# jcbowden/EagleEverything

Measured on NVIDIA B200. Metric: markers/s, higher is better.
Workload: dtype f64

## Files before the change

eagleeverything_b200/csrc/capi.cu:

```cuda
#include <cublas_v2.h>
#include <dlfcn.h>
#include <fcntl.h>
#include <sys/mman.h>
#include <sys/stat.h>
#include <unistd.h>

#include <cmath>
#include <cstdarg>
#include <cstdlib>
#include <cstring>
#include <atomic>
#include <condition_variable>
#include <functional>
#include <mutex>
#include <thread>
#include <unordered_map>
#include <string>
#include <vector>

#include "common.cuh"
#include "hostio.cuh"

struct eg_store {
    int8_t* d = nullptr;
// ... 82 lines not shown
    if (g_ctx.ready) return check_cuda(cudaSetDevice(g_ctx.device), "cudaSetDevice");
    const char* env = getenv("EAGLE_GPU_DEVICE");
    return eg_init(env ? atoi(env) : 0);
}

int ensure_init_pub() { return ensure_init(); }
cudaStream_t ctx_stream() { return g_ctx.stream; }
cublasHandle_t ctx_cublas() { return g_ctx.cublas; }

void syrk_release_cache();
void scan_i8_release();
void algebra_release();
void eigbasis_release();
void prep_i8_release();
int launch_prepare_i8(const double* d_S, const double* d_V, int64_t n, int64_t col0, int64_t col1, double* d_tmp,
                      double* d_Wp, int64_t Kpad, cudaStream_t st, bool* done);
static int g_scan_mode = -1;
int scan_mode() {
    if (g_scan_mode < 0) {
        const char* e = getenv("EAGLE_SCAN_MODE");
        g_scan_mode = (e && (e[0] == 'f' || e[0] == 'd' || e[0] == '0')) ? 0 : 1;
    }
    return g_scan_mode;
}
int launch_scan(const int8_t* d_Mt, int64_t L, int64_t n, int64_t pitch, const double* d_Wp,
                const int64_t* d_zero_rows, int n_zero, double* d_a, double* d_vara, cudaStream_t st);

static void pool_flush_locked() {
    for (auto& b : g_ctx.free_blocks) cudaFreeAsync(b.p, g_ctx.stream);
    g_ctx.free_blocks.clear();
    g_ctx.free_bytes = 0;
// ... 422 lines not shown
    __shared__ int8_t tile[32][33];
    const int tx = threadIdx.x & 31, ty = threadIdx.x >> 5;
    const int64_t r0 = (int64_t)blockIdx.y * 32, c0 = (int64_t)blockIdx.x * 32;
    for (int i = ty; i < 32; i += 8) {
        const int64_t r = r0 + i, c = c0 + tx;
        tile[i][tx] = (r < rows && c < cols) ? in[r * pitch + c] : (int8_t)0;
    }
    __syncthreads();
    for (int i = ty; i < 32; i += 8) {
        const int64_t c = c0 + i, r = r0 + tx;
        if (r < rows && c < cols) out[r + c * rows] = -(double)tile[tx][i];
    }
}

__global__ void __launch_bounds__(256) symmetrize_upper_kernel(double* __restrict__ Wp, int64_t n, int64_t ld,
                                                               int w_is_upper) {
    __shared__ double tile[32][33];
    const int bx = blockIdx.x, by = blockIdx.y;
    if (bx < by) return;
    const int tx = threadIdx.x & 31, ty = threadIdx.x >> 5;
    const int64_t r0 = (int64_t)by * 32, c0 = (int64_t)bx * 32;
    for (int i = ty; i < 32; i += 8) {
        const int64_t r = c0 + tx, c = r0 + i;
        tile[i][tx] = (r < n && c < n) ? Wp[r + c * ld] : 0.0;
    }
    __syncthreads();
    for (int i = ty; i < 32; i += 8) {
        const int64_t r = r0 + tx, c = c0 + i;
        if (r < n && c < n) {
            if (r < c) Wp[r + c * ld] = Wp[r + c * ld] + (w_is_upper ? Wp[r + c * ld] : tile[tx][i]);
            else if (r > c) Wp[r + c * ld] = 0.0;
        }
    }
    if (bx != by) {
        __syncthreads();
        for (int i = ty; i < 32; i += 8) {
            const int64_t r = c0 + tx, c = r0 + i;
            if (r < n && c < n) Wp[r + c * ld] = 0.0;
        }
    }
}

__global__ void __launch_bounds__(256) symmetry_kernel(const double* __restrict__ A, int64_t n,
                                                       unsigned long long* __restrict__ out) {
    __shared__ double tile[64][65];
// ... 25 lines not shown
            const double a = v[k], b = tile[tx][i];
            mabs = fmax(mabs, fmax(fabs(a), fabs(b)));
            const double d = fabs(a - b);
            masym = fmax(masym, d == d ? d : 1.0e300);
        }
    }
#pragma unroll
    for (int o = 16; o > 0; o >>= 1) {
        mabs = fmax(mabs, __shfl_xor_sync(0xffffffffu, mabs, o));
        masym = fmax(masym, __shfl_xor_sync(0xffffffffu, masym, o));
    }
    if ((threadIdx.x & 31) == 0) {
        atomicMax(out, (unsigned long long)__double_as_longlong(mabs));
        atomicMax(out + 1, (unsigned long long)__double_as_longlong(masym));
    }
}

static void say(eg_message_fn message, void* ctx, const char* fmt, ...) {
    if (!message) return;
    char buf[512];
    va_list ap;
    va_start(ap, fmt);
    vsnprintf(buf, sizeof(buf), fmt, ap);
    va_end(ap);
    message(ctx, buf);
}

}

using namespace eg;
// ... 371 lines not shown
    MTRACE("scan: upload of 1/%d of S and V", N);
    EG_TRY(agree(upload()));
    if (N > 1) {
        EG_NCCL(g_nccl.GroupStart());
        for (int q = 0; q < N; q++) {
            int64_t q0, q1;
            shard_range(n, N, q, 1, &q0, &q1);
            if (q1 == q0) continue;
            EG_NCCL(g_nccl.Broadcast(dS.as<double>() + q0 * n, dS.as<double>() + q0 * n, (size_t)(q1 - q0) * n, NCCL_FLOAT64, q, g_multi.comm[r], st));
            EG_NCCL(g_nccl.Broadcast(dV.as<double>() + q0 * n, dV.as<double>() + q0 * n, (size_t)(q1 - q0) * n, NCCL_FLOAT64, q, g_multi.comm[r], st));
        }
        EG_NCCL(g_nccl.GroupEnd());
    }
    g_ctx.timing[4] = t_up.stop();
    Timer t_prep(st);
    int sym = 0;
    bool split = false;
    std::vector<int64_t> cuts(N + 1, n);
    auto products = [&]() -> int {
        EG_TRY(eg_dev_inputs_symmetric(dS.as<double>(), dV.as<double>(), n, &sym, st));
        split = sym && eg_prep_uses_i8(n);
        for (int q = 0; q < N; q++) {
            if (split) {
                int64_t c = (int64_t)llround((double)n * (sqrt(1.0 + 3.0 * q / N) - 1.0) / 32.0) * 32;
                cuts[q] = c < n ? c : n;
            } else {
                cuts[q] = q == 0 ? 0 : n;
            }
        }
        int64_t widest = 1;
        for (int q = 0; q < N; q++) widest = std::max(widest, cuts[q + 1] - cuts[q]);
        EG_TRY(dT.alloc((size_t)n * (split ? widest : n) * 8, "scan scratch"));
        EG_CUDA(cudaMemsetAsync(dW.p, 0, (size_t)eg_scan_wp_elems(n) * 8, st));
        return eg_dev_scan_prepare_cols(dS.as<double>(), dV.as<double>(), n, split ? cuts[r] : 0, split ? cuts[r + 1] : n, sym,
                                        dT.as<double>(), dW.as<double>(), st);
    };
    MTRACE("scan: pre-products of my columns of W");
    EG_TRY(agree(products()));
    if (N > 1) {
        EG_NCCL(g_nccl.GroupStart());
        for (int q = 0; q < N && split; q++)
            if (cuts[q + 1] > cuts[q])
                EG_NCCL(g_nccl.Broadcast(dW.as<double>() + cuts[q] * Kpad, dW.as<double>() + cuts[q] * Kpad,
                                         (size_t)(cuts[q + 1] - cuts[q]) * Kpad, NCCL_FLOAT64, q, g_multi.comm[r], st));
        EG_NCCL(g_nccl.GroupEnd());
    }
    EG_TRY(eg_dev_scan_fold(dS.as<double>(), da.as<double>(), n, sym, dW.as<double>(), st));
    g_ctx.timing[5] = t_prep.stop();
    MTRACE("scan: %lld markers", (long long)L);
    if (L > 0) {
        const std::vector<int64_t> z = slot_indices(Mt, r, zero_rows);
        {
            Timer t(st);
            EG_TRY(eg_dev_scan(part->d, L, n, part->pitch, dW.as<double>(), z.empty() ? nullptr : z.data(), (int64_t)z.size(),
                               oa.as<double>(), ov.as<double>(), st));
            g_ctx.timing[6] = t.stop();
        }
        Timer t(st);
        EG_CUDA(cudaMemcpyAsync(out_a + Mt->off[r], oa.p, (size_t)L * 8, cudaMemcpyDeviceToHost, st));
        EG_CUDA(cudaMemcpyAsync(out_vara + Mt->off[r], ov.p, (size_t)L * 8, cudaMemcpyDeviceToHost, st));
        EG_CUDA(cudaStreamSynchronize(st));
        g_ctx.timing[7] = t.stop();
// ... 373 lines not shown
    if (env_pm && env_pm[0] == 'f') return 0;
    return n >= 512;
}

extern "C" int eg_dev_scan_prepare_cols(const double* d_S, const double* d_V, int64_t n, int64_t col0, int64_t col1,
                                        int upper_only, double* d_tmp, double* d_Wp, void* stream) {
    if (!d_S || !d_V || !d_tmp || !d_Wp || n <= 0 || col0 < 0 || col1 > n || col0 > col1)
        return set_error(EG_ERR_ARG, "eg_dev_scan_prepare_cols: bad argument");
    if (col0 == col1) return EG_OK;
    EG_TRY(ensure_init());
    cudaStream_t st = (cudaStream_t)stream;
    const int64_t Kpad = round_up(n, 32), nc = col1 - col0;
    const bool want_i8 = eg_prep_uses_i8(n) != 0;
    if (upper_only && want_i8) {
        bool done = false;
        EG_TRY(launch_prepare_i8(d_S, d_V, n, col0, col1, d_tmp, d_Wp, Kpad, st, &done));
        if (done) return EG_OK;
    }
    const double one = 1.0, zero = 0.0;
    if (cublasSetStream(g_ctx.cublas, st) != CUBLAS_STATUS_SUCCESS) return set_error(EG_ERR_CUDA, "cublasSetStream");
    if (cublasDgemm(g_ctx.cublas, CUBLAS_OP_N, CUBLAS_OP_N, (int)n, (int)nc, (int)n, &one, d_V, (int)n, d_S + col0 * n,
                    (int)n, &zero, d_tmp, (int)n) != CUBLAS_STATUS_SUCCESS)
        return set_error(EG_ERR_CUDA, "cublasDgemm(V*S) failed");
    const int64_t step = upper_only ? 1024 : nc;
    for (int64_t b0 = 0; b0 < nc; b0 += step) {
        const int64_t nb = (b0 + step <= nc) ? step : nc - b0;
        const int64_t rows = upper_only ? (col0 + b0 + nb) : n;
        if (cublasDgemm(g_ctx.cublas, CUBLAS_OP_N, CUBLAS_OP_N, (int)rows, (int)nb, (int)n, &one, d_S, (int)n,
                        d_tmp + b0 * n, (int)n, &zero, d_Wp + (col0 + b0) * Kpad, (int)Kpad) != CUBLAS_STATUS_SUCCESS)
            return set_error(EG_ERR_CUDA, "cublasDgemm(S*tmp) failed");
    }
    return EG_OK;
}

extern "C" int eg_dev_scan_fold(const double* d_S, const double* d_a, int64_t n, int w_is_upper, double* d_Wp,
                                void* stream) {
    if (!d_S || !d_a || !d_Wp || n <= 0) return set_error(EG_ERR_ARG, "eg_dev_scan_fold: bad argument");
    EG_TRY(ensure_init());
    cudaStream_t st = (cudaStream_t)stream;
    const int64_t Kpad = round_up(n, 32);
    const double one = 1.0, zero = 0.0;
    if (cublasSetStream(g_ctx.cublas, st) != CUBLAS_STATUS_SUCCESS) return set_error(EG_ERR_CUDA, "cublasSetStream");
    if (cublasDgemv(g_ctx.cublas, CUBLAS_OP_N, (int)n, (int)n, &one, d_S, (int)n, d_a, 1, &zero, d_Wp + n * Kpad, 1) !=
        CUBLAS_STATUS_SUCCESS)
        return set_error(EG_ERR_CUDA, "cublasDgemv(S*a) failed");
    const unsigned nb = (unsigned)((n + 31) / 32);
    symmetrize_upper_kernel<<<dim3(nb, nb), 256, 0, st>>>(d_Wp, n, Kpad, w_is_upper);
    return check_launch("symmetrize_upper_kernel");
}

extern "C" int eg_dev_inputs_symmetric(const double* d_S, const double* d_V, int64_t n, int* yes, void* stream) {
    if (!yes) return set_error(EG_ERR_ARG, "null");
    double aS, dS, aV, dV;
    EG_TRY(eg_dev_symmetry(d_S, n, &aS, &dS, stream));
    EG_TRY(eg_dev_symmetry(d_V, n, &aV, &dV, stream));
    const char* env = getenv("EAGLE_SCAN_SYMMETRIC");
    *yes = !(env && env[0] == '0') && dS <= 1e-13 * aS && dV <= 1e-13 * aV;
    return EG_OK;
}

extern "C" int eg_dev_scan_prepare(const double* d_S, const double* d_V, const double* d_a, int64_t n, double* d_tmp,
                                   double* d_Wp, void* stream) {
    if (!d_S || !d_V || !d_a || !d_tmp || !d_Wp || n <= 0) return set_error(EG_ERR_ARG, "eg_dev_scan_prepare: bad argument");
    EG_TRY(ensure_init());
    int sym = 0;
    EG_TRY(eg_dev_inputs_symmetric(d_S, d_V, n, &sym, stream));
    EG_CUDA(cudaMemsetAsync(d_Wp, 0, (size_t)eg_scan_wp_elems(n) * 8, (cudaStream_t)stream));
    EG_TRY(eg_dev_scan_prepare_cols(d_S, d_V, n, 0, n, sym, d_tmp, d_Wp, stream));
    return eg_dev_scan_fold(d_S, d_a, n, sym, d_Wp, stream);
}

extern "C" int eg_ReadBlock(const char* asciifname, int64_t start_row, int64_t numcols, int64_t numrows_in_block,
                            double* out_colmajor) {
    if (!asciifname || !out_colmajor || start_row < 0 || numcols <= 0 || numrows_in_block <= 0)
        return set_error(EG_ERR_ARG, "ReadBlock: bad argument");
    EG_TRY(ensure_init());
    MappedFile f;
    EG_TRY(f.open_ro(asciifname));
    const void* nl = memchr(f.p, '\n', f.size);
    const int64_t line = nl ? (const uint8_t*)nl - f.p : (int64_t)f.size;
    if (numcols > line) return set_error(EG_ERR_FORMAT, "ReadBlock: lines of %s have %lld characters, %lld requested",
                                         asciifname, (long long)line, (long long)numcols);
    const int64_t nrows_file = ((int64_t)f.size + 1) / (line + 1);
    if (start_row + numrows_in_block > nrows_file)
// ... 641 lines not shown
```

eagleeverything_b200/csrc/prep_i8.cu:

```cuda
#include <cstdlib>
#include <vector>

#include "common.cuh"
#include "ptx.cuh"

namespace eg {

constexpr int PI_BM = 128;
constexpr int PI_BN = 256;
constexpr int PI_BK = 128;
constexpr int PI_STAGES = 4;
constexpr int PI_A_BYTES = PI_BM * PI_BK;
constexpr int PI_B_BYTES = PI_BN * PI_BK;
constexpr int PI_STAGE_BYTES = PI_A_BYTES + PI_B_BYTES;
constexpr int PI_THREADS = 192;
constexpr int PI_TMEM_COLS = 512;
constexpr int PI_SLICES = 7;
constexpr int PI_LEVELS = 7;
constexpr int PI_TERMS = PI_LEVELS * (PI_LEVELS + 1) / 2;
constexpr int PI_SMEM_BYTES = PI_STAGES * PI_STAGE_BYTES + 1024 + 256;
constexpr int PI_SROWS = 12;
constexpr int PI_PHASE = 8;
constexpr int PI_LAG = 4;

// ... 1 lines not shown
    int64_t M, N, ld;
    double* out;
    const double* sL;
    const double* sR;
    int32_t lrow0, rrow0;
    int32_t KB;
    int64_t diag_shift;
    int32_t upper_only;
    const int2* tiles;
    int32_t ntiles, nchunks, ngroups;
    uint8_t tp[PI_TERMS], tq[PI_TERMS];
    uint8_t cbeg[PI_TERMS + 1];
    double cw[PI_TERMS];
    uint32_t* phase_ctr;
    int32_t phases_per_tile, phase_len, lag;
};

__device__ __forceinline__ void pi_red_add(uint32_t* p, uint32_t v) {
    asm volatile("red.relaxed.gpu.global.add.u32 [%0], %1;" ::"l"(p), "r"(v) : "memory");
}
__device__ __forceinline__ uint32_t pi_ld(const uint32_t* p) {
    uint32_t v;
    asm volatile("ld.relaxed.gpu.global.u32 %0, [%1];" : "=r"(v) : "l"(p) : "memory");
    return v;
}

__global__ void __launch_bounds__(PI_THREADS, 1)
prep_i8_kernel(const __grid_constant__ CUtensorMap tmapL, const __grid_constant__ CUtensorMap tmapR, const PrepParams p) {
    extern __shared__ uint8_t smem_raw[];
    uint8_t* smem = reinterpret_cast<uint8_t*>((reinterpret_cast<uintptr_t>(smem_raw) + 1023) & ~(uintptr_t)1023);
    uint64_t* bars = reinterpret_cast<uint64_t*>(smem + PI_STAGES * PI_STAGE_BYTES);
    uint64_t* full = bars;
    uint64_t* empty = bars + PI_STAGES;
    uint64_t* tmem_full = bars + 2 * PI_STAGES;
    uint64_t* tmem_empty = tmem_full + 2;
    uint32_t* tmem_slot = reinterpret_cast<uint32_t*>(tmem_empty + 2);

    const int warp = threadIdx.x >> 5, lane = threadIdx.x & 31;
    if (warp == 0 && lane == 0) {
        ptx::prefetch_tmap(&tmapL);
        ptx::prefetch_tmap(&tmapR);
        for (int s = 0; s < PI_STAGES; s++) {
            ptx::mbar_init(&full[s], 1);
            ptx::mbar_init(&empty[s], 1);
        }
        for (int a = 0; a < 2; a++) {
            ptx::mbar_init(&tmem_full[a], 1);
            ptx::mbar_init(&tmem_empty[a], 4);
        }
        ptx::fence_mbar_init();
    }
    if (warp == 1) ptx::tmem_alloc<PI_TMEM_COLS>(tmem_slot);
// ... 154 lines not shown
constexpr int PP_STAGE_BYTES = PI_A_BYTES + PP_B_BYTES;
constexpr int PP_SMEM_BYTES = PP_STAGES * PP_STAGE_BYTES + 1024 + 256;
constexpr int PP_BM = 2 * PI_BM;

__global__ void __launch_bounds__(PI_THREADS, 1)
prep_i8_pair_kernel(const __grid_constant__ CUtensorMap tmapL, const __grid_constant__ CUtensorMap tmapR, const PrepParams p) {
    extern __shared__ uint8_t smem_raw[];
    uint8_t* smem = reinterpret_cast<uint8_t*>((reinterpret_cast<uintptr_t>(smem_raw) + 1023) & ~(uintptr_t)1023);
    uint64_t* bars = reinterpret_cast<uint64_t*>(smem + PP_STAGES * PP_STAGE_BYTES);
    uint64_t* full = bars;
    uint64_t* empty = bars + PP_STAGES;
    uint64_t* tmem_full = bars + 2 * PP_STAGES;
    uint64_t* tmem_empty = tmem_full + 2;
    uint32_t* tmem_slot = reinterpret_cast<uint32_t*>(tmem_empty + 2);

    const int warp = threadIdx.x >> 5, lane = threadIdx.x & 31;
    const uint32_t rank = ptx::cluster_ctarank();
    const int cid = (int)ptx::cluster_id_x();
    const int ncl = (int)gridDim.x / 2;
    if (warp == 0 && lane == 0) {
        ptx::prefetch_tmap(&tmapL);
        ptx::prefetch_tmap(&tmapR);
        for (int s = 0; s < PP_STAGES; s++) {
            ptx::mbar_init(&full[s], 1);
            ptx::mbar_init(&empty[s], 1);
        }
        for (int a = 0; a < 2; a++) {
            ptx::mbar_init(&tmem_full[a], 1);
            ptx::mbar_init(&tmem_empty[a], 8);
        }
// ... 140 lines not shown
            ptx::tc_fence_before();
            __syncwarp();
            if (lane == 0) ptx::mbar_arrive_cluster(ptx::mapa(ptx::smem_u32(&tmem_empty[acc]), 0));
            if (++acc == 2) { acc = 0; acc_phase ^= 1; }
        }
    }

    ptx::tc_fence_before();
    ptx::cluster_sync();
    if (warp == 1) {
        ptx::tc_fence_after();
        ptx::tmem_dealloc_pair<PI_TMEM_COLS>(tmem_base);
    }
}

__global__ void __launch_bounds__(256) pi_colscale_kernel(const double* __restrict__ A, int64_t rows, int64_t ld,
                                                          int32_t* __restrict__ expo, double* __restrict__ scale,
                                                          const double* __restrict__ rowscale) {
    const int64_t c = blockIdx.x;
    unsigned long long m = 0;
    for (int64_t i = threadIdx.x; i < rows; i += 256) {
        const double x = rowscale ? A[i + c * ld] * rowscale[i] : A[i + c * ld];
        const unsigned long long b = (unsigned long long)__double_as_longlong(x) & 0x7FFFFFFFFFFFFFFFull;
        m = b > m ? b : m;
    }
    __shared__ unsigned long long sh[8];
#pragma unroll
    for (int o = 16; o > 0; o >>= 1) {
        const unsigned long long other = __shfl_xor_sync(0xffffffffu, m, o);
        m = other > m ? other : m;
    }
    if ((threadIdx.x & 31) == 0) sh[threadIdx.x >> 5] = m;
    __syncthreads();
    if (threadIdx.x == 0) {
        for (int w = 1; w < 8; w++) m = sh[w] > m ? sh[w] : m;
        const double amax = __longlong_as_double((long long)m);
        int e = 0;
        double s = 0.0;
        if (m >= 0x7FF0000000000000ull) {
            s = __longlong_as_double(0x7FF8000000000000LL);
        } else if (amax > 0.0) {
            if (frexp(amax, &e) >= 0.9921875) e++;
            s = ldexp(1.0, e - 55);
        }
        expo[c] = e;
        scale[c] = s;
    }
}
__global__ void __launch_bounds__(256) pi_slice_kernel(const double* __restrict__ A, int64_t rows, int64_t ld,
                                                       const int32_t* __restrict__ expo, int8_t* __restrict__ Q, int64_t Kp,
                                                       int64_t slice_stride, const double* __restrict__ rowscale) {
    const int64_t c = blockIdx.y;
    const int64_t i0 = ((int64_t)blockIdx.x * 256 + threadIdx.x) * 4;
    if (i0 >= Kp) return;
    uint32_t out[PI_SLICES];
#pragma unroll
    for (int s = 0; s < PI_SLICES; s++) out[s] = 0;
    const int e = expo[c];
#pragma unroll
    for (int d = 0; d < 4; d++) {
        const int64_t i = i0 + d;
        if (i < rows) {
            const double xs = ldexp(rowscale ? A[i + c * ld] * rowscale[i] : A[i + c * ld], 55 - e);
            long long X = fabs(xs) < 3.6e16 ? __double2ll_rn(xs) : 0;
#pragma unroll
            for (int s = PI_SLICES - 1; s > 0; s--) {
                const int q = (int)(int8_t)(X & 0xFF);
                out[s] |= ((uint32_t)q & 0xFFu) << (8 * d);
                X = (X - q) >> 8;
            }
            out[0] |= ((uint32_t)(int)X & 0xFFu) << (8 * d);
        }
    }
    int8_t* base = Q + c * Kp + i0;
#pragma unroll
    for (int s = 0; s < PI_SLICES; s++) *reinterpret_cast<uint32_t*>(base + (int64_t)s * slice_stride) = out[s];
}

// ... 25 lines not shown
    return EG_OK;
}

static bool prep_i8_pair() {
    const char* e = getenv("EAGLE_PREP_PAIR");
    return e && e[0] == '1';
}

struct PrepWorkspace {
    int device = -1;
    int8_t* qS = nullptr;  size_t qS_cap = 0;
    int8_t* qV = nullptr;  size_t qV_cap = 0;
    int8_t* qX = nullptr;  size_t qX_cap = 0;
    double* sc = nullptr;  size_t sc_cap = 0;
    int32_t* ex = nullptr; size_t ex_cap = 0;
    int2* tiles = nullptr; size_t tiles_cap = 0;
    uint32_t* phase = nullptr; size_t phase_cap = 0;
};
static thread_local PrepWorkspace g_pi;

static thread_local cudaEvent_t g_pi_ev[4] = {nullptr, nullptr, nullptr, nullptr};
static thread_local double g_pi_ops = 0.0;
static thread_local int g_pi_marks = 0;
void prep_kernel_times(double* ms, double* ops) {
    *ms = 0.0;
    *ops = g_pi_ops;
    for (int i = 0; i + 1 < g_pi_marks; i += 2) {
        float f = 0.f;
        if (cudaEventSynchronize(g_pi_ev[i + 1]) == cudaSuccess && cudaEventElapsedTime(&f, g_pi_ev[i], g_pi_ev[i + 1]) == cudaSuccess)
            *ms += f;
    }
}

void prep_i8_release() {
    cudaFree(g_pi.qS); cudaFree(g_pi.qV); cudaFree(g_pi.qX); cudaFree(g_pi.sc); cudaFree(g_pi.ex); cudaFree(g_pi.tiles); cudaFree(g_pi.phase);
    g_pi = PrepWorkspace();
}
template <class T>
static bool pi_grow(T** ptr, size_t* cap, size_t need) {
    if (need <= *cap && *ptr) return true;
    if (*ptr) cudaFree(*ptr);
    *ptr = nullptr;
    *cap = 0;
    if (malloc_retry((void**)ptr, need * sizeof(T)) != cudaSuccess) {
        cudaGetLastError();
        return false;
    }
    *cap = need;
    return true;
}

static int pi_slice(const double* d_A, int64_t rows, int64_t ld, int64_t ncols, int8_t* Q, int64_t Kp, int32_t* expo,
                    double* scale, cudaStream_t st, const double* d_rowscale = nullptr) {
    pi_colscale_kernel<<<(unsigned)ncols, 256, 0, st>>>(d_A, rows, ld, expo, scale, d_rowscale);
    EG_TRY(check_launch("pi_colscale_kernel"));
    pi_slice_kernel<<<dim3((unsigned)((Kp / 4 + 255) / 256), (unsigned)ncols), 256, 0, st>>>(d_A, rows, ld, expo, Q, Kp,
                                                                                          Kp * ncols, d_rowscale);
    return check_launch("pi_slice_kernel");
}

static int pi_product(const int8_t* qL, int64_t lrows, const double* sL, int64_t lrow0, int64_t M, const int8_t* qR,
                      int64_t rrows, const double* sR, int64_t rrow0, int64_t N, int64_t n, int64_t Kp, double* out,
                      int64_t ld, bool upper_only, int64_t diag_shift, cudaStream_t st) {
    const bool pair = prep_i8_pair();
    const int BMt = pair ? PP_BM : PI_BM;
    const int TM = (int)((M + BMt - 1) / BMt), TN = (int)((N + PI_BN - 1) / PI_BN);
    std::vector<int2> h;
    int srows = PI_SROWS;
    if (const char* e = getenv("EAGLE_PREP_SROWS")) srows = atoi(e) > 0 ? atoi(e) : srows;
    if (pair) srows = (srows + 1) / 2;
    for (int sr = 0; sr < TM; sr += srows)
        for (int tj = 0; tj < TN; tj++)
            for (int ti = sr; ti < TM && ti < sr + srows; ti++) {
                if (upper_only && (int64_t)(tj + 1) * PI_BN - 1 + diag_shift < (int64_t)ti * BMt) continue;
                h.push_back(make_int2(ti, tj));
            }
    if (h.empty()) return EG_OK;
    if (!pi_grow(&g_pi.tiles, &g_pi.tiles_cap, h.size())) return set_error(EG_ERR_ALLOC, "prep_i8: tile table");
    EG_CUDA(cudaMemcpyAsync(g_pi.tiles, h.data(), h.size() * sizeof(int2), cudaMemcpyHostToDevice, st));
    EG_CUDA(cudaStreamSynchronize(st));

    PrepParams p;
    p.M = M; p.N = N; p.ld = ld; p.out = out;
    p.sL = sL + lrow0; p.sR = sR + rrow0;
    p.lrow0 = (int32_t)lrow0; p.rrow0 = (int32_t)rrow0;
    p.KB = (int32_t)(Kp / PI_BK);
    p.diag_shift = diag_shift;
    p.upper_only = upper_only ? 1 : 0;
    p.tiles = g_pi.tiles;
    p.ntiles = (int32_t)h.size();
    const int64_t tmax64 = (((int64_t)1 << 31) - 1) / (n * 16384);
    const int tmax = (int)(tmax64 > PI_LEVELS ? PI_LEVELS : tmax64);
    if (tmax < 1) return set_error(EG_ERR_ARG, "prep_i8: n = %lld too large for int32 accumulation", (long long)n);
    int nt = 0, nc = 0;
    for (int d = PI_LEVELS - 1; d >= 0; d--) {
        for (int p0 = 0; p0 <= d; p0 += tmax) {
            p.cbeg[nc] = (uint8_t)nt;
            double w = 1.0;
            for (int e = 0; e < PI_LEVELS - 1 - d; e++) w *= 256.0;
            p.cw[nc] = w;
            for (int pp = p0; pp <= d && pp < p0 + tmax; pp++) {
                p.tp[nt] = (uint8_t)pp;
                p.tq[nt] = (uint8_t)(d - pp);
                nt++;
            }
// ... 30 lines not shown
    cudaLaunchConfig_t cfg = {};
    cfg.gridDim = dim3((unsigned)grid);
    cfg.blockDim = dim3(PI_THREADS);
    cfg.dynamicSmemBytes = pair ? PP_SMEM_BYTES : PI_SMEM_BYTES;
    cfg.stream = st;
    cudaLaunchAttribute attr[2];
    attr[0].id = cudaLaunchAttributeCooperative;
    attr[0].val.cooperative = flow ? 1 : 0;
    attr[1].id = cudaLaunchAttributeClusterDimension;
    attr[1].val.clusterDim.x = 2;
    attr[1].val.clusterDim.y = 1;
    attr[1].val.clusterDim.z = 1;
    cfg.attrs = attr;
    cfg.numAttrs = pair ? 2 : 1;
    if (!g_pi_ev[0])
        for (int i = 0; i < 4; i++) cudaEventCreate(&g_pi_ev[i]);
    if (g_pi_marks <= 2) {
        cudaEventRecord(g_pi_ev[g_pi_marks], st);
        g_pi_ops += (double)p.ntiles * nt * p.KB * 2.0 * BMt * PI_BN * PI_BK;
    }
    if (pair) EG_CUDA(cudaLaunchKernelEx(&cfg, prep_i8_pair_kernel, tL, tR, p));
    else EG_CUDA(cudaLaunchKernelEx(&cfg, prep_i8_kernel, tL, tR, p));
    if (g_pi_marks <= 2) {
        cudaEventRecord(g_pi_ev[g_pi_marks + 1], st);
        g_pi_marks += 2;
    }
    return check_launch("prep_i8_kernel");
}

int launch_prepare_i8(const double* d_S, const double* d_V, int64_t n, int64_t col0, int64_t col1, double* d_tmp,
                      double* d_Wp, int64_t Kpad, cudaStream_t st, bool* done) {
    *done = false;
    g_pi_marks = 0;
    g_pi_ops = 0.0;
    int dev = 0;
    EG_CUDA(cudaGetDevice(&dev));
    if (g_pi.device != dev) {
        if (g_pi.device >= 0) prep_i8_release();
        g_pi.device = dev;
    }
    if (n * 16384 >= ((int64_t)1 << 31)) return EG_OK;
    const int64_t Kp = round_up(n, 128), nc = col1 - col0;
    size_t free_b = 0, total_b = 0;
    EG_CUDA(cudaMemGetInfo(&free_b, &total_b));
    const size_t need = (size_t)PI_SLICES * Kp * (size_t)(2 * n + nc);
    const size_t have = g_pi.qS_cap + g_pi.qV_cap + g_pi.qX_cap;
    if (need > have && need - have + ((size_t)2 << 30) > free_b) return EG_OK;
    if (!pi_grow(&g_pi.qS, &g_pi.qS_cap, (size_t)PI_SLICES * Kp * n) || !pi_grow(&g_pi.qV, &g_pi.qV_cap, (size_t)PI_SLICES * Kp * n) ||
        !pi_grow(&g_pi.qX, &g_pi.qX_cap, (size_t)PI_SLICES * Kp * nc) || !pi_grow(&g_pi.sc, &g_pi.sc_cap, (size_t)(2 * n + nc)) ||
        !pi_grow(&g_pi.ex, &g_pi.ex_cap, (size_t)(2 * n + nc)))
        return EG_OK;
    double *sS = g_pi.sc, *sV = g_pi.sc + n, *sX = g_pi.sc + 2 * n;
    int32_t *eS = g_pi.ex, *eV = g_pi.ex + n, *eX = g_pi.ex + 2 * n;
    EG_TRY(pi_slice(d_S, n, n, n, g_pi.qS, Kp, eS, sS, st));
    EG_TRY(pi_slice(d_V, n, n, n, g_pi.qV, Kp, eV, sV, st));
    EG_TRY(pi_product(g_pi.qV, n, sV, 0, n, g_pi.qS, n, sS, col0, nc, n, Kp, d_tmp, n, false, 0, st));
    EG_TRY(pi_slice(d_tmp, n, n, nc, g_pi.qX, Kp, eX, sX, st));
    EG_TRY(pi_product(g_pi.qS, n, sS, 0, col1, g_pi.qX, nc, sX, 0, nc, n, Kp, d_Wp + col0 * Kpad, Kpad, true, col0, st));
    *done = true;
    return EG_OK;
}

int launch_prepare_eig_i8(const double* d_Ut, const double* d_rs, int64_t n, double* d_Wp, int64_t Kpad, cudaStream_t st,
                          bool* done) {
    *done = false;
    g_pi_marks = 0;
    g_pi_ops = 0.0;
    int dev = 0;
    EG_CUDA(cudaGetDevice(&dev));
    if (g_pi.device != dev) {
        if (g_pi.device >= 0) prep_i8_release();
        g_pi.device = dev;
    }
    if (n * 16384 >= ((int64_t)1 << 31)) return EG_OK;
    const int64_t Kp = round_up(n, 128);
    size_t free_b = 0, total_b = 0;
    EG_CUDA(cudaMemGetInfo(&free_b, &total_b));
    const size_t need = (size_t)PI_SLICES * Kp * (size_t)n;
    if (need > g_pi.qS_cap && need - g_pi.qS_cap + ((size_t)2 << 30) > free_b) return EG_OK;
    if (!pi_grow(&g_pi.qS, &g_pi.qS_cap, need) || !pi_grow(&g_pi.sc, &g_pi.sc_cap, (size_t)n) ||
        !pi_grow(&g_pi.ex, &g_pi.ex_cap, (size_t)n))
        return EG_OK;
    EG_TRY(pi_slice(d_Ut, n, n, n, g_pi.qS, Kp, g_pi.ex, g_pi.sc, st, d_rs));
    EG_TRY(pi_product(g_pi.qS, n, g_pi.sc, 0, n, g_pi.qS, n, g_pi.sc, 0, n, n, Kp, d_Wp, Kpad, true, 0, st));
    *done = true;
    return EG_OK;
}

}
```

eagleeverything_b200/device.py:

```python
from __future__ import annotations

import ctypes as C

import numpy as np
import torch

from . import _lib


def _ptr(t):
    return C.c_void_p(t.data_ptr())


def _stream():
    return C.c_void_p(torch.cuda.current_stream().cuda_stream)


def store_pitch(cols: int) -> int:
    return (cols + 1 + 127) // 128 * 128


def init(device: int):
    lib = _lib.require_gpu()
    torch.cuda.set_device(device)
# ... 96 lines not shown
    return Wp


def scan_prepare_sharded(S, V, a, n, rank, world, Wp=None, tmp=None):
    import torch.distributed as dist
    lib = _lib.load()
    Kpad = (n + 31) // 32 * 32
    if Wp is None:
        Wp = torch.empty(lib.eg_scan_wp_elems(n), dtype=torch.float64, device=S.device)
    sym = C.c_int(0)
    _lib.check(lib.eg_dev_inputs_symmetric(_ptr(S), _ptr(V), n, C.byref(sym), _stream()))
    sym = int(sym.value)
    if not (sym and lib.eg_prep_uses_i8(n)):
        if tmp is None or tmp.numel() < n * n:
            tmp = torch.empty(n * n, dtype=torch.float64, device=S.device)
        Wp.zero_()
        _lib.check(lib.eg_dev_scan_prepare_cols(_ptr(S), _ptr(V), n, 0, n, sym, _ptr(tmp), _ptr(Wp), _stream()))
        _lib.check(lib.eg_dev_scan_fold(_ptr(S), _ptr(a), n, sym, _ptr(Wp), _stream()))
        return Wp
    if sym:
        cuts = [min(n, int(round(n * ((1.0 + 3.0 * r / world) ** 0.5 - 1.0) / 32.0)) * 32) for r in range(world)] + [n]
    else:
        blk = (n + world - 1) // world
        cuts = [min(r * blk, n) for r in range(world)] + [n]
    c0, c1 = cuts[rank], cuts[rank + 1]
    need = n * max(max(cuts[r + 1] - cuts[r] for r in range(world)), 1)
    if tmp is None or tmp.numel() < need:
        tmp = torch.empty(need, dtype=torch.float64, device=S.device)
    Wp.zero_()
    _lib.check(lib.eg_dev_scan_prepare_cols(_ptr(S), _ptr(V), n, c0, c1, sym, _ptr(tmp), _ptr(Wp), _stream()))
    Wv = Wp[: (Wp.numel() // Kpad) * Kpad].view(-1, Kpad)
    sizes = [(cuts[r + 1] - cuts[r]) * cuts[r + 1] for r in range(world)]
    smax = max(sizes)
    if (world + 1) * smax * 8 <= (4 << 30):
        mine = torch.zeros(smax, dtype=torch.float64, device=S.device)
        if c1 > c0:
            mine[: sizes[rank]].view(c1 - c0, c1).copy_(Wv[c0:c1, :c1])
        allb = torch.empty(world * smax, dtype=torch.float64, device=S.device)
        dist.all_gather_into_tensor(allb, mine)
# ... 45 lines not shown
```

Before: 2.898 million.

## Decide input symmetry on device and gate prep kernels to avoid host syncs

Result: no change. 2.944 million (median of 6 runs) (+1.6%).

```diff
diff --git a/eagleeverything_b200/csrc/capi.cu b/eagleeverything_b200/csrc/capi.cu
--- a/eagleeverything_b200/csrc/capi.cu
+++ b/eagleeverything_b200/csrc/capi.cu
@@ -120,7 +120,7 @@
 void eigbasis_release();
 void prep_i8_release();
 int launch_prepare_i8(const double* d_S, const double* d_V, int64_t n, int64_t col0, int64_t col1, double* d_tmp,
-                      double* d_Wp, int64_t Kpad, cudaStream_t st, bool* done);
+                      double* d_Wp, int64_t Kpad, const int* d_sym, cudaStream_t st, bool* done);
 static int g_scan_mode = -1;
 int scan_mode() {
     if (g_scan_mode < 0) {
@@ -573,8 +573,9 @@
 }
 
 __global__ void __launch_bounds__(256) symmetrize_upper_kernel(double* __restrict__ Wp, int64_t n, int64_t ld,
-                                                               int w_is_upper) {
+                                                               int w_is_upper, const int* __restrict__ d_w_is_upper) {
     __shared__ double tile[32][33];
+    const bool upper = d_w_is_upper ? *d_w_is_upper != 0 : w_is_upper != 0;
     const int bx = blockIdx.x, by = blockIdx.y;
     if (bx < by) return;
     const int tx = threadIdx.x & 31, ty = threadIdx.x >> 5;
@@ -587,7 +588,7 @@
     for (int i = ty; i < 32; i += 8) {
         const int64_t r = r0 + tx, c = c0 + i;
         if (r < n && c < n) {
-            if (r < c) Wp[r + c * ld] = Wp[r + c * ld] + (w_is_upper ? Wp[r + c * ld] : tile[tx][i]);
+            if (r < c) Wp[r + c * ld] = Wp[r + c * ld] + (upper ? Wp[r + c * ld] : tile[tx][i]);
             else if (r > c) Wp[r + c * ld] = 0.0;
         }
     }
@@ -643,6 +644,68 @@
         atomicMax(out, (unsigned long long)__double_as_longlong(mabs));
         atomicMax(out + 1, (unsigned long long)__double_as_longlong(masym));
     }
+}
+
+__global__ void sym_decide_kernel(const unsigned long long* __restrict__ m, int allowed, int* __restrict__ sym) {
+    const double aS = __longlong_as_double((long long)m[0]), dS = __longlong_as_double((long long)m[1]);
+    const double aV = __longlong_as_double((long long)m[2]), dV = __longlong_as_double((long long)m[3]);
+    *sym = allowed && dS <= 1e-13 * aS && dV <= 1e-13 * aV;
+}
+static bool symmetric_allowed() {
+    const char* env = getenv("EAGLE_SCAN_SYMMETRIC");
+    return !(env && env[0] == '0');
+}
+
+struct ScanSym {
+    int host = 0;
+    int* dev = nullptr;
+    void* ws = nullptr;
+    cudaStream_t st = nullptr;
+    ScanSym() = default;
+    ScanSym(const ScanSym&) = delete;
+    ScanSym& operator=(const ScanSym&) = delete;
+    ~ScanSym() { release(); }
+    void release() {
+        if (ws) scratch_free(ws, st);
+        ws = nullptr;
+        dev = nullptr;
+    }
+};
+
+static int scan_products(const double* d_S, const double* d_V, int64_t n, int64_t col0, int64_t col1, double* d_tmp,
+                         double* d_Wp, cudaStream_t st, ScanSym* sym) {
+    sym->st = st;
+    if (eg_prep_uses_i8(n) && scratch_alloc(&sym->ws, 4 * sizeof(unsigned long long) + sizeof(int), st) == cudaSuccess) {
+        unsigned long long* m = static_cast<unsigned long long*>(sym->ws);
+        sym->dev = reinterpret_cast<int*>(m + 4);
+        EG_CUDA(cudaMemsetAsync(m, 0, 4 * sizeof(unsigned long long), st));
+        const unsigned nb = (unsigned)((n + 63) / 64);
+        symmetry_kernel<<<dim3(nb, nb), 256, 0, st>>>(d_S, n, m);
+        EG_TRY(check_launch("symmetry_kernel"));
+        symmetry_kernel<<<dim3(nb, nb), 256, 0, st>>>(d_V, n, m + 2);
+        EG_TRY(check_launch("symmetry_kernel"));
+        sym_decide_kernel<<<1, 1, 0, st>>>(m, symmetric_allowed() ? 1 : 0, sym->dev);
+        EG_TRY(check_launch("sym_decide_kernel"));
+        bool done = col0 == col1;
+        if (!done) EG_TRY(launch_prepare_i8(d_S, d_V, n, col0, col1, d_tmp, d_Wp, round_up(n, 32), sym->dev, st, &done));
+        if (done) return EG_OK;
+        sym->release();
+    }
+    EG_TRY(eg_dev_inputs_symmetric(d_S, d_V, n, &sym->host, st));
+    return eg_dev_scan_prepare_cols(d_S, d_V, n, col0, col1, sym->host, d_tmp, d_Wp, st);
+}
+
+static int scan_fold(const double* d_S, const double* d_a, int64_t n, int w_is_upper, const int* d_w_is_upper, double* d_Wp,
+                     cudaStream_t st) {
+    const int64_t Kpad = round_up(n, 32);
+    const double one = 1.0, zero = 0.0;
+    if (cublasSetStream(g_ctx.cublas, st) != CUBLAS_STATUS_SUCCESS) return set_error(EG_ERR_CUDA, "cublasSetStream");
+    if (cublasDgemv(g_ctx.cublas, CUBLAS_OP_N, (int)n, (int)n, &one, d_S, (int)n, d_a, 1, &zero, d_Wp + n * Kpad, 1) !=
+        CUBLAS_STATUS_SUCCESS)
+        return set_error(EG_ERR_CUDA, "cublasDgemv(S*a) failed");
+    const unsigned nb = (unsigned)((n + 31) / 32);
+    symmetrize_upper_kernel<<<dim3(nb, nb), 256, 0, st>>>(d_Wp, n, Kpad, w_is_upper, d_w_is_upper);
+    return check_launch("symmetrize_upper_kernel");
 }
 
 static void say(eg_message_fn message, void* ctx, const char* fmt, ...) {
@@ -1044,12 +1107,11 @@
     }
     g_ctx.timing[4] = t_up.stop();
     Timer t_prep(st);
-    int sym = 0;
+    ScanSym sym;
     bool split = false;
     std::vector<int64_t> cuts(N + 1, n);
     auto products = [&]() -> int {
-        EG_TRY(eg_dev_inputs_symmetric(dS.as<double>(), dV.as<double>(), n, &sym, st));
-        split = sym && eg_prep_uses_i8(n);
+        split = eg_prep_uses_i8(n) != 0;
         for (int q = 0; q < N; q++) {
             if (split) {
                 int64_t c = (int64_t)llround((double)n * (sqrt(1.0 + 3.0 * q / N) - 1.0) / 32.0) * 32;
@@ -1062,8 +1124,8 @@
         for (int q = 0; q < N; q++) widest = std::max(widest, cuts[q + 1] - cuts[q]);
         EG_TRY(dT.alloc((size_t)n * (split ? widest : n) * 8, "scan scratch"));
         EG_CUDA(cudaMemsetAsync(dW.p, 0, (size_t)eg_scan_wp_elems(n) * 8, st));
-        return eg_dev_scan_prepare_cols(dS.as<double>(), dV.as<double>(), n, split ? cuts[r] : 0, split ? cuts[r + 1] : n, sym,
-                                        dT.as<double>(), dW.as<double>(), st);
+        return scan_products(dS.as<double>(), dV.as<double>(), n, split ? cuts[r] : 0, split ? cuts[r + 1] : n,
+                             dT.as<double>(), dW.as<double>(), st, &sym);
     };
     MTRACE("scan: pre-products of my columns of W");
     EG_TRY(agree(products()));
@@ -1075,7 +1137,7 @@
                                          (size_t)(cuts[q + 1] - cuts[q]) * Kpad, NCCL_FLOAT64, q, g_multi.comm[r], st));
         EG_NCCL(g_nccl.GroupEnd());
     }
-    EG_TRY(eg_dev_scan_fold(dS.as<double>(), da.as<double>(), n, sym, dW.as<double>(), st));
+    EG_TRY(scan_fold(dS.as<double>(), da.as<double>(), n, sym.host, sym.dev, dW.as<double>(), st));
     g_ctx.timing[5] = t_prep.stop();
     MTRACE("scan: %lld markers", (long long)L);
     if (L > 0) {
@@ -1479,7 +1541,7 @@
     const bool want_i8 = eg_prep_uses_i8(n) != 0;
     if (upper_only && want_i8) {
         bool done = false;
-        EG_TRY(launch_prepare_i8(d_S, d_V, n, col0, col1, d_tmp, d_Wp, Kpad, st, &done));
+        EG_TRY(launch_prepare_i8(d_S, d_V, n, col0, col1, d_tmp, d_Wp, Kpad, nullptr, st, &done));
         if (done) return EG_OK;
     }
     const double one = 1.0, zero = 0.0;
@@ -1502,16 +1564,7 @@
                                 void* stream) {
     if (!d_S || !d_a || !d_Wp || n <= 0) return set_error(EG_ERR_ARG, "eg_dev_scan_fold: bad argument");
     EG_TRY(ensure_init());
-    cudaStream_t st = (cudaStream_t)stream;
-    const int64_t Kpad = round_up(n, 32);
-    const double one = 1.0, zero = 0.0;
-    if (cublasSetStream(g_ctx.cublas, st) != CUBLAS_STATUS_SUCCESS) return set_error(EG_ERR_CUDA, "cublasSetStream");
-    if (cublasDgemv(g_ctx.cublas, CUBLAS_OP_N, (int)n, (int)n, &one, d_S, (int)n, d_a, 1, &zero, d_Wp + n * Kpad, 1) !=
-        CUBLAS_STATUS_SUCCESS)
-        return set_error(EG_ERR_CUDA, "cublasDgemv(S*a) failed");
-    const unsigned nb = (unsigned)((n + 31) / 32);
-    symmetrize_upper_kernel<<<dim3(nb, nb), 256, 0, st>>>(d_Wp, n, Kpad, w_is_upper);
-    return check_launch("symmetrize_upper_kernel");
+    return scan_fold(d_S, d_a, n, w_is_upper, nullptr, d_Wp, (cudaStream_t)stream);
 }
 
 extern "C" int eg_dev_inputs_symmetric(const double* d_S, const double* d_V, int64_t n, int* yes, void* stream) {
@@ -1519,8 +1572,7 @@
     double aS, dS, aV, dV;
     EG_TRY(eg_dev_symmetry(d_S, n, &aS, &dS, stream));
     EG_TRY(eg_dev_symmetry(d_V, n, &aV, &dV, stream));
-    const char* env = getenv("EAGLE_SCAN_SYMMETRIC");
-    *yes = !(env && env[0] == '0') && dS <= 1e-13 * aS && dV <= 1e-13 * aV;
+    *yes = symmetric_allowed() && dS <= 1e-13 * aS && dV <= 1e-13 * aV;
     return EG_OK;
 }
 
@@ -1528,11 +1580,11 @@
                                    double* d_Wp, void* stream) {
     if (!d_S || !d_V || !d_a || !d_tmp || !d_Wp || n <= 0) return set_error(EG_ERR_ARG, "eg_dev_scan_prepare: bad argument");
     EG_TRY(ensure_init());
-    int sym = 0;
-    EG_TRY(eg_dev_inputs_symmetric(d_S, d_V, n, &sym, stream));
-    EG_CUDA(cudaMemsetAsync(d_Wp, 0, (size_t)eg_scan_wp_elems(n) * 8, (cudaStream_t)stream));
-    EG_TRY(eg_dev_scan_prepare_cols(d_S, d_V, n, 0, n, sym, d_tmp, d_Wp, stream));
-    return eg_dev_scan_fold(d_S, d_a, n, sym, d_Wp, stream);
+    cudaStream_t st = (cudaStream_t)stream;
+    EG_CUDA(cudaMemsetAsync(d_Wp, 0, (size_t)eg_scan_wp_elems(n) * 8, st));
+    ScanSym sym;
+    EG_TRY(scan_products(d_S, d_V, n, 0, n, d_tmp, d_Wp, st, &sym));
+    return scan_fold(d_S, d_a, n, sym.host, sym.dev, d_Wp, st);
 }
 
 extern "C" int eg_ReadBlock(const char* asciifname, int64_t start_row, int64_t numcols, int64_t numrows_in_block,
diff --git a/eagleeverything_b200/csrc/prep_i8.cu b/eagleeverything_b200/csrc/prep_i8.cu
--- a/eagleeverything_b200/csrc/prep_i8.cu
+++ b/eagleeverything_b200/csrc/prep_i8.cu
@@ -39,6 +39,8 @@
     double cw[PI_TERMS];
     uint32_t* phase_ctr;
     int32_t phases_per_tile, phase_len, lag;
+    const int* sym;
+    int32_t run_if_sym;
 };
 
 __device__ __forceinline__ void pi_red_add(uint32_t* p, uint32_t v) {
@@ -61,6 +63,7 @@
     uint64_t* tmem_empty = tmem_full + 2;
     uint32_t* tmem_slot = reinterpret_cast<uint32_t*>(tmem_empty + 2);
 
+    if (p.sym && (*p.sym != 0) != (p.run_if_sym != 0)) return;
     const int warp = threadIdx.x >> 5, lane = threadIdx.x & 31;
     if (warp == 0 && lane == 0) {
         ptx::prefetch_tmap(&tmapL);
@@ -245,6 +248,7 @@
     uint64_t* tmem_empty = tmem_full + 2;
     uint32_t* tmem_slot = reinterpret_cast<uint32_t*>(tmem_empty + 2);
 
+    if (p.sym && (*p.sym != 0) != (p.run_if_sym != 0)) return;
     const int warp = threadIdx.x >> 5, lane = threadIdx.x & 31;
     const uint32_t rank = ptx::cluster_ctarank();
     const int cid = (int)ptx::cluster_id_x();
@@ -415,13 +419,22 @@
     }
 }
 
+__device__ __forceinline__ bool pi_by_rows(const int* sym) { return sym && *sym == 0; }
+__device__ __forceinline__ double pi_elem(const double* A, int64_t i, int64_t c, int64_t ld, const double* rowscale,
+                                          bool by_rows) {
+    if (by_rows) return A[c + i * ld];
+    return rowscale ? A[i + c * ld] * rowscale[i] : A[i + c * ld];
+}
 __global__ void __launch_bounds__(256) pi_colscale_kernel(const double* __restrict__ A, int64_t rows, int64_t ld,
                                                           int32_t* __restrict__ expo, double* __restrict__ scale,
-                                                          const double* __restrict__ rowscale) {
+                                                          const double* __restrict__ rowscale, const int* __restrict__ sym,
+                                                          int asym_only) {
+    const bool by_rows = pi_by_rows(sym);
+    if (asym_only && !by_rows) return;
     const int64_t c = blockIdx.x;
     unsigned long long m = 0;
     for (int64_t i = threadIdx.x; i < rows; i += 256) {
-        const double x = rowscale ? A[i + c * ld] * rowscale[i] : A[i + c * ld];
+        const double x = pi_elem(A, i, c, ld, rowscale, by_rows);
         const unsigned long long b = (unsigned long long)__double_as_longlong(x) & 0x7FFFFFFFFFFFFFFFull;
         m = b > m ? b : m;
     }
@@ -450,7 +463,10 @@
 }
 __global__ void __launch_bounds__(256) pi_slice_kernel(const double* __restrict__ A, int64_t rows, int64_t ld,
                                                        const int32_t* __restrict__ expo, int8_t* __restrict__ Q, int64_t Kp,
-                                                       int64_t slice_stride, const double* __restrict__ rowscale) {
+                                                       int64_t slice_stride, const double* __restrict__ rowscale,
+                                                       const int* __restrict__ sym, int asym_only) {
+    const bool by_rows = pi_by_rows(sym);
+    if (asym_only && !by_rows) return;
     const int64_t c = blockIdx.y;
     const int64_t i0 = ((int64_t)blockIdx.x * 256 + threadIdx.x) * 4;
     if (i0 >= Kp) return;
@@ -462,7 +478,7 @@
     for (int d = 0; d < 4; d++) {
         const int64_t i = i0 + d;
         if (i < rows) {
-            const double xs = ldexp(rowscale ? A[i + c * ld] * rowscale[i] : A[i + c * ld], 55 - e);
+            const double xs = ldexp(pi_elem(A, i, c, ld, rowscale, by_rows), 55 - e);
             long long X = fabs(xs) < 3.6e16 ? __double2ll_rn(xs) : 0;
 #pragma unroll
             for (int s = PI_SLICES - 1; s > 0; s--) {
@@ -518,27 +534,50 @@
     int8_t* qX = nullptr;  size_t qX_cap = 0;
     double* sc = nullptr;  size_t sc_cap = 0;
     int32_t* ex = nullptr; size_t ex_cap = 0;
-    int2* tiles = nullptr; size_t tiles_cap = 0;
     uint32_t* phase = nullptr; size_t phase_cap = 0;
+    int* sym = nullptr;    size_t sym_cap = 0;
 };
 static thread_local PrepWorkspace g_pi;
 
-static thread_local cudaEvent_t g_pi_ev[4] = {nullptr, nullptr, nullptr, nullptr};
-static thread_local double g_pi_ops = 0.0;
-static thread_local int g_pi_marks = 0;
+struct PrepTiles {
+    int device;
+    int64_t M, N, diag_shift;
+    int bm, srows;
+    bool upper_only;
+    int2* d;
+    int count;
+};
+static thread_local std::vector<PrepTiles> g_pi_tiles;
+
+constexpr int PI_MAX_LAUNCHES = 3;
+static thread_local cudaEvent_t g_pi_ev[2 * PI_MAX_LAUNCHES] = {};
+static thread_local double g_pi_ops[PI_MAX_LAUNCHES] = {};
+static thread_local int g_pi_gate[PI_MAX_LAUNCHES] = {};
+static thread_local int g_pi_launches = 0;
 void prep_kernel_times(double* ms, double* ops) {
     *ms = 0.0;
-    *ops = g_pi_ops;
-    for (int i = 0; i + 1 < g_pi_marks; i += 2) {
-        float f = 0.f;
-        if (cudaEventSynchronize(g_pi_ev[i + 1]) == cudaSuccess && cudaEventElapsedTime(&f, g_pi_ev[i], g_pi_ev[i + 1]) == cudaSuccess)
-            *ms += f;
+    *ops = 0.0;
+    float f[PI_MAX_LAUNCHES] = {};
+    bool gated = false;
+    for (int i = 0; i < g_pi_launches; i++) {
+        if (cudaEventSynchronize(g_pi_ev[2 * i + 1]) != cudaSuccess || cudaEventElapsedTime(&f[i], g_pi_ev[2 * i], g_pi_ev[2 * i + 1]) != cudaSuccess)
+            f[i] = 0.f;
+        gated |= g_pi_gate[i] >= 0;
+    }
+    int sym = -1;
+    if (gated && g_pi.sym && cudaMemcpy(&sym, g_pi.sym, sizeof(int), cudaMemcpyDeviceToHost) != cudaSuccess) sym = -1;
+    for (int i = 0; i < g_pi_launches; i++) {
+        if (g_pi_gate[i] >= 0 && g_pi_gate[i] != (sym != 0)) continue;
+        *ms += f[i];
+        *ops += g_pi_ops[i];
     }
 }
 
 void prep_i8_release() {
-    cudaFree(g_pi.qS); cudaFree(g_pi.qV); cudaFree(g_pi.qX); cudaFree(g_pi.sc); cudaFree(g_pi.ex); cudaFree(g_pi.tiles); cudaFree(g_pi.phase);
+    cudaFree(g_pi.qS); cudaFree(g_pi.qV); cudaFree(g_pi.qX); cudaFree(g_pi.sc); cudaFree(g_pi.ex); cudaFree(g_pi.phase); cudaFree(g_pi.sym);
     g_pi = PrepWorkspace();
+    for (PrepTiles& t : g_pi_tiles) cudaFree(t.d);
+    g_pi_tiles.clear();
 }
 template <class T>
 static bool pi_grow(T** ptr, size_t* cap, size_t need) {
@@ -555,34 +594,64 @@
 }
 
 static int pi_slice(const double* d_A, int64_t rows, int64_t ld, int64_t ncols, int8_t* Q, int64_t Kp, int32_t* expo,
-                    double* scale, cudaStream_t st, const double* d_rowscale = nullptr) {
-    pi_colscale_kernel<<<(unsigned)ncols, 256, 0, st>>>(d_A, rows, ld, expo, scale, d_rowscale);
+                    double* scale, cudaStream_t st, const double* d_rowscale = nullptr, const int* d_sym = nullptr,
+                    bool asym_only = false) {
+    pi_colscale_kernel<<<(unsigned)ncols, 256, 0, st>>>(d_A, rows, ld, expo, scale, d_rowscale, d_sym, asym_only);
     EG_TRY(check_launch("pi_colscale_kernel"));
     pi_slice_kernel<<<dim3((unsigned)((Kp / 4 + 255) / 256), (unsigned)ncols), 256, 0, st>>>(d_A, rows, ld, expo, Q, Kp,
-                                                                                          Kp * ncols, d_rowscale);
+                                                                                          Kp * ncols, d_rowscale, d_sym,
+                                                                                          asym_only);
     return check_launch("pi_slice_kernel");
+}
+
+static int pi_tiles(int64_t M, int64_t N, bool upper_only, int64_t diag_shift, int bm, int srows, cudaStream_t st,
+                    const PrepTiles** out) {
+    int dev = 0;
+    EG_CUDA(cudaGetDevice(&dev));
+    for (const PrepTiles& t : g_pi_tiles)
+        if (t.device == dev && t.M == M && t.N == N && t.upper_only == upper_only && t.diag_shift == diag_shift &&
+            t.bm == bm && t.srows == srows) {
+            *out = &t;
+            return EG_OK;
+        }
+    const int TM = (int)((M + bm - 1) / bm), TN = (int)((N + PI_BN - 1) / PI_BN);
+    std::vector<int2> h;
+    for (int sr = 0; sr < TM; sr += srows)
+        for (int tj = 0; tj < TN; tj++)
+            for (int ti = sr; ti < TM && ti < sr + srows; ti++) {
+                if (upper_only && (int64_t)(tj + 1) * PI_BN - 1 + diag_shift < (int64_t)ti * bm) continue;
+                h.push_back(make_int2(ti, tj));
+            }
+    if (g_pi_tiles.size() >= 32) {
+        for (PrepTiles& t : g_pi_tiles) cudaFree(t.d);
+        g_pi_tiles.clear();
+    }
+    PrepTiles t = {dev, M, N, diag_shift, bm, srows, upper_only, nullptr, (int)h.size()};
+    if (!h.empty() && malloc_retry((void**)&t.d, h.size() * sizeof(int2)) != cudaSuccess) {
+        cudaGetLastError();
+        return set_error(EG_ERR_ALLOC, "prep_i8: tile table");
+    }
+    g_pi_tiles.push_back(t);
+    if (!h.empty()) {
+        EG_CUDA(cudaMemcpyAsync(t.d, h.data(), h.size() * sizeof(int2), cudaMemcpyHostToDevice, st));
+        EG_CUDA(cudaStreamSynchronize(st));
+    }
+    *out = &g_pi_tiles.back();
+    return EG_OK;
 }
 
 static int pi_product(const int8_t* qL, int64_t lrows, const double* sL, int64_t lrow0, int64_t M, const int8_t* qR,
                       int64_t rrows, const double* sR, int64_t rrow0, int64_t N, int64_t n, int64_t Kp, double* out,
-                      int64_t ld, bool upper_only, int64_t diag_shift, cudaStream_t st) {
+                      int64_t ld, bool upper_only, int64_t diag_shift, cudaStream_t st, const int* d_sym = nullptr,
+                      int run_if_sym = 1) {
     const bool pair = prep_i8_pair();
     const int BMt = pair ? PP_BM : PI_BM;
-    const int TM = (int)((M + BMt - 1) / BMt), TN = (int)((N + PI_BN - 1) / PI_BN);
-    std::vector<int2> h;
     int srows = PI_SROWS;
     if (const char* e = getenv("EAGLE_PREP_SROWS")) srows = atoi(e) > 0 ? atoi(e) : srows;
     if (pair) srows = (srows + 1) / 2;
-    for (int sr = 0; sr < TM; sr += srows)
-        for (int tj = 0; tj < TN; tj++)
-            for (int ti = sr; ti < TM && ti < sr + srows; ti++) {
-                if (upper_only && (int64_t)(tj + 1) * PI_BN - 1 + diag_shift < (int64_t)ti * BMt) continue;
-                h.push_back(make_int2(ti, tj));
-            }
-    if (h.empty()) return EG_OK;
-    if (!pi_grow(&g_pi.tiles, &g_pi.tiles_cap, h.size())) return set_error(EG_ERR_ALLOC, "prep_i8: tile table");
-    EG_CUDA(cudaMemcpyAsync(g_pi.tiles, h.data(), h.size() * sizeof(int2), cudaMemcpyHostToDevice, st));
-    EG_CUDA(cudaStreamSynchronize(st));
+    const PrepTiles* tiles = nullptr;
+    EG_TRY(pi_tiles(M, N, upper_only, diag_shift, BMt, srows, st, &tiles));
+    if (tiles->count == 0) return EG_OK;
 
     PrepParams p;
     p.M = M; p.N = N; p.ld = ld; p.out = out;
@@ -591,8 +660,10 @@
     p.KB = (int32_t)(Kp / PI_BK);
     p.diag_shift = diag_shift;
     p.upper_only = upper_only ? 1 : 0;
-    p.tiles = g_pi.tiles;
-    p.ntiles = (int32_t)h.size();
+    p.tiles = tiles->d;
+    p.ntiles = (int32_t)tiles->count;
+    p.sym = d_sym;
+    p.run_if_sym = run_if_sym;
     const int64_t tmax64 = (((int64_t)1 << 31) - 1) / (n * 16384);
     const int tmax = (int)(tmax64 > PI_LEVELS ? PI_LEVELS : tmax64);
     if (tmax < 1) return set_error(EG_ERR_ARG, "prep_i8: n = %lld too large for int32 accumulation", (long long)n);
@@ -653,25 +724,23 @@
     cfg.attrs = attr;
     cfg.numAttrs = pair ? 2 : 1;
     if (!g_pi_ev[0])
-        for (int i = 0; i < 4; i++) cudaEventCreate(&g_pi_ev[i]);
-    if (g_pi_marks <= 2) {
-        cudaEventRecord(g_pi_ev[g_pi_marks], st);
-        g_pi_ops += (double)p.ntiles * nt * p.KB * 2.0 * BMt * PI_BN * PI_BK;
+        for (int i = 0; i < 2 * PI_MAX_LAUNCHES; i++) cudaEventCreate(&g_pi_ev[i]);
+    const int slot = g_pi_launches < PI_MAX_LAUNCHES ? g_pi_launches++ : -1;
+    if (slot >= 0) {
+        cudaEventRecord(g_pi_ev[2 * slot], st);
+        g_pi_ops[slot] = (double)p.ntiles * nt * p.KB * 2.0 * BMt * PI_BN * PI_BK;
+        g_pi_gate[slot] = d_sym ? run_if_sym : -1;
     }
     if (pair) EG_CUDA(cudaLaunchKernelEx(&cfg, prep_i8_pair_kernel, tL, tR, p));
     else EG_CUDA(cudaLaunchKernelEx(&cfg, prep_i8_kernel, tL, tR, p));
-    if (g_pi_marks <= 2) {
-        cudaEventRecord(g_pi_ev[g_pi_marks + 1], st);
-        g_pi_marks += 2;
-    }
+    if (slot >= 0) cudaEventRecord(g_pi_ev[2 * slot + 1], st);
     return check_launch("prep_i8_kernel");
 }
 
 int launch_prepare_i8(const double* d_S, const double* d_V, int64_t n, int64_t col0, int64_t col1, double* d_tmp,
-                      double* d_Wp, int64_t Kpad, cudaStream_t st, bool* done) {
+                      double* d_Wp, int64_t Kpad, const int* d_sym, cudaStream_t st, bool* done) {
     *done = false;
-    g_pi_marks = 0;
-    g_pi_ops = 0.0;
+    g_pi_launches = 0;
     int dev = 0;
     EG_CUDA(cudaGetDevice(&dev));
     if (g_pi.device != dev) {
@@ -680,22 +749,31 @@
     }
     if (n * 16384 >= ((int64_t)1 << 31)) return EG_OK;
     const int64_t Kp = round_up(n, 128), nc = col1 - col0;
-    size_t free_b = 0, total_b = 0;
-    EG_CUDA(cudaMemGetInfo(&free_b, &total_b));
-    const size_t need = (size_t)PI_SLICES * Kp * (size_t)(2 * n + nc);
-    const size_t have = g_pi.qS_cap + g_pi.qV_cap + g_pi.qX_cap;
-    if (need > have && need - have + ((size_t)2 << 30) > free_b) return EG_OK;
-    if (!pi_grow(&g_pi.qS, &g_pi.qS_cap, (size_t)PI_SLICES * Kp * n) || !pi_grow(&g_pi.qV, &g_pi.qV_cap, (size_t)PI_SLICES * Kp * n) ||
-        !pi_grow(&g_pi.qX, &g_pi.qX_cap, (size_t)PI_SLICES * Kp * nc) || !pi_grow(&g_pi.sc, &g_pi.sc_cap, (size_t)(2 * n + nc)) ||
-        !pi_grow(&g_pi.ex, &g_pi.ex_cap, (size_t)(2 * n + nc)))
-        return EG_OK;
+    const size_t qn = (size_t)PI_SLICES * Kp * n, qx = (size_t)PI_SLICES * Kp * nc, ns = (size_t)(2 * n + nc);
+    if (qn > g_pi.qS_cap || qn > g_pi.qV_cap || qx > g_pi.qX_cap || ns > g_pi.sc_cap || ns > g_pi.ex_cap || !g_pi.sym) {
+        size_t free_b = 0, total_b = 0;
+        EG_CUDA(cudaMemGetInfo(&free_b, &total_b));
+        const size_t need = qn * 2 + qx;
+        const size_t have = g_pi.qS_cap + g_pi.qV_cap + g_pi.qX_cap;
+        if (need > have && need - have + ((size_t)2 << 30) > free_b) return EG_OK;
+        if (!pi_grow(&g_pi.qS, &g_pi.qS_cap, qn) || !pi_grow(&g_pi.qV, &g_pi.qV_cap, qn) || !pi_grow(&g_pi.qX, &g_pi.qX_cap, qx) ||
+            !pi_grow(&g_pi.sc, &g_pi.sc_cap, ns) || !pi_grow(&g_pi.ex, &g_pi.ex_cap, ns) || !pi_grow(&g_pi.sym, &g_pi.sym_cap, 1))
+            return EG_OK;
+    }
     double *sS = g_pi.sc, *sV = g_pi.sc + n, *sX = g_pi.sc + 2 * n;
     int32_t *eS = g_pi.ex, *eV = g_pi.ex + n, *eX = g_pi.ex + 2 * n;
+    if (d_sym) EG_CUDA(cudaMemcpyAsync(g_pi.sym, d_sym, sizeof(int), cudaMemcpyDeviceToDevice, st));
     EG_TRY(pi_slice(d_S, n, n, n, g_pi.qS, Kp, eS, sS, st));
-    EG_TRY(pi_slice(d_V, n, n, n, g_pi.qV, Kp, eV, sV, st));
+    EG_TRY(pi_slice(d_V, n, n, n, g_pi.qV, Kp, eV, sV, st, nullptr, d_sym));
     EG_TRY(pi_product(g_pi.qV, n, sV, 0, n, g_pi.qS, n, sS, col0, nc, n, Kp, d_tmp, n, false, 0, st));
     EG_TRY(pi_slice(d_tmp, n, n, nc, g_pi.qX, Kp, eX, sX, st));
-    EG_TRY(pi_product(g_pi.qS, n, sS, 0, col1, g_pi.qX, nc, sX, 0, nc, n, Kp, d_Wp + col0 * Kpad, Kpad, true, col0, st));
+    EG_TRY(pi_product(g_pi.qS, n, sS, 0, col1, g_pi.qX, nc, sX, 0, nc, n, Kp, d_Wp + col0 * Kpad, Kpad, true, col0, st,
+                      d_sym, 1));
+    if (d_sym) {
+        EG_TRY(pi_slice(d_S, n, n, n, g_pi.qS, Kp, eS, sS, st, nullptr, d_sym, true));
+        EG_TRY(pi_product(g_pi.qS, n, sS, 0, n, g_pi.qX, nc, sX, 0, nc, n, Kp, d_Wp + col0 * Kpad, Kpad, false, 0, st,
+                          d_sym, 0));
+    }
     *done = true;
     return EG_OK;
 }
@@ -703,8 +781,7 @@
 int launch_prepare_eig_i8(const double* d_Ut, const double* d_rs, int64_t n, double* d_Wp, int64_t Kpad, cudaStream_t st,
                           bool* done) {
     *done = false;
-    g_pi_marks = 0;
-    g_pi_ops = 0.0;
+    g_pi_launches = 0;
     int dev = 0;
     EG_CUDA(cudaGetDevice(&dev));
     if (g_pi.device != dev) {
@@ -713,13 +790,15 @@
     }
     if (n * 16384 >= ((int64_t)1 << 31)) return EG_OK;
     const int64_t Kp = round_up(n, 128);
-    size_t free_b = 0, total_b = 0;
-    EG_CUDA(cudaMemGetInfo(&free_b, &total_b));
     const size_t need = (size_t)PI_SLICES * Kp * (size_t)n;
-    if (need > g_pi.qS_cap && need - g_pi.qS_cap + ((size_t)2 << 30) > free_b) return EG_OK;
-    if (!pi_grow(&g_pi.qS, &g_pi.qS_cap, need) || !pi_grow(&g_pi.sc, &g_pi.sc_cap, (size_t)n) ||
-        !pi_grow(&g_pi.ex, &g_pi.ex_cap, (size_t)n))
-        return EG_OK;
+    if (need > g_pi.qS_cap || (size_t)n > g_pi.sc_cap || (size_t)n > g_pi.ex_cap) {
+        size_t free_b = 0, total_b = 0;
+        EG_CUDA(cudaMemGetInfo(&free_b, &total_b));
+        if (need > g_pi.qS_cap && need - g_pi.qS_cap + ((size_t)2 << 30) > free_b) return EG_OK;
+        if (!pi_grow(&g_pi.qS, &g_pi.qS_cap, need) || !pi_grow(&g_pi.sc, &g_pi.sc_cap, (size_t)n) ||
+            !pi_grow(&g_pi.ex, &g_pi.ex_cap, (size_t)n))
+            return EG_OK;
+    }
     EG_TRY(pi_slice(d_Ut, n, n, n, g_pi.qS, Kp, g_pi.ex, g_pi.sc, st, d_rs));
     EG_TRY(pi_product(g_pi.qS, n, g_pi.sc, 0, n, g_pi.qS, n, g_pi.sc, 0, n, n, Kp, d_Wp, Kpad, true, 0, st));
     *done = true;
diff --git a/eagleeverything_b200/device.py b/eagleeverything_b200/device.py
--- a/eagleeverything_b200/device.py
+++ b/eagleeverything_b200/device.py
@@ -134,15 +134,9 @@
     if not (sym and lib.eg_prep_uses_i8(n)):
         if tmp is None or tmp.numel() < n * n:
             tmp = torch.empty(n * n, dtype=torch.float64, device=S.device)
-        Wp.zero_()
-        _lib.check(lib.eg_dev_scan_prepare_cols(_ptr(S), _ptr(V), n, 0, n, sym, _ptr(tmp), _ptr(Wp), _stream()))
-        _lib.check(lib.eg_dev_scan_fold(_ptr(S), _ptr(a), n, sym, _ptr(Wp), _stream()))
+        _lib.check(lib.eg_dev_scan_prepare(_ptr(S), _ptr(V), _ptr(a), n, _ptr(tmp), _ptr(Wp), _stream()))
         return Wp
-    if sym:
-        cuts = [min(n, int(round(n * ((1.0 + 3.0 * r / world) ** 0.5 - 1.0) / 32.0)) * 32) for r in range(world)] + [n]
-    else:
-        blk = (n + world - 1) // world
-        cuts = [min(r * blk, n) for r in range(world)] + [n]
+    cuts = [min(n, int(round(n * ((1.0 + 3.0 * r / world) ** 0.5 - 1.0) / 32.0)) * 32) for r in range(world)] + [n]
     c0, c1 = cuts[rank], cuts[rank + 1]
     need = n * max(max(cuts[r + 1] - cuts[r] for r in range(world)), 1)
     if tmp is None or tmp.numel() < need:
```
